# dluvizon/deephar

Measured on NVIDIA H100. Metric: frames/sec (256x256, 16-frame clips, b32), higher is better.
Workload: dtype bf16x3 split (fp32 accumulate, wgmma)

## Files before the change

deephar_b200/_ffi.py:

```python
import ctypes as C
import os

_HERE = os.path.dirname(os.path.abspath(__file__))
LIB_PATH = os.environ.get('DEEPHAR_B200_LIB') or os.path.join(_HERE, 'libdeephar_b200.so')


class DeepharB200Error(RuntimeError):
    pass


class dh_view(C.Structure):
    _fields_ = [('p', C.c_void_p), ('n', C.c_int32), ('h', C.c_int32), ('w', C.c_int32),
                ('c', C.c_int32), ('ld', C.c_int32)]


class dh_conv_desc(C.Structure):
    _fields_ = [('kh', C.c_int32), ('kw', C.c_int32), ('sh', C.c_int32), ('sw', C.c_int32),
                ('pad_same', C.c_int32), ('pre_relu', C.c_int32), ('post_relu', C.c_int32),
                ('n_res', C.c_int32),
                ('pre_scale', C.c_void_p), ('pre_shift', C.c_void_p),
                ('post_scale', C.c_void_p), ('post_shift', C.c_void_p),
                ('res', dh_view * 2),
                ('precision', C.c_int32), ('res_up2x', C.c_int32), ('pool_out', dh_view)]


class dh_frame_src(C.Structure):
    _fields_ = [('data', C.c_uint64), ('h', C.c_int32), ('w', C.c_int32), ('stride', C.c_int32),
                ('x0', C.c_int32), ('y0', C.c_int32), ('cw', C.c_int32), ('ch', C.c_int32), ('hflip', C.c_int32),
                ('kx_off', C.c_int32), ('ky_off', C.c_int32), ('kx_coef_off', C.c_int32), ('ky_coef_off', C.c_int32),
                ('ksx', C.c_int32), ('ksy', C.c_int32)]


class dh_frame_box(C.Structure):
    _fields_ = [('data', C.c_uint64), ('h', C.c_int32), ('w', C.c_int32), ('stride', C.c_int32),
                ('hflip', C.c_int32), ('objpos', C.c_double * 2), ('winsize', C.c_double * 2)]


FRAME_EMPTY, FRAME_TOO_LARGE, FRAME_BAD_BOX = 1, 2, 4


class dh_packed_w(C.Structure):
    _fields_ = [('hi', C.c_void_p), ('lo', C.c_void_p), ('cout_pad', C.c_int32), ('k', C.c_int32)]


class dh_conv_plan_info(C.Structure):
    _fields_ = [('path', C.c_int32), ('fallback', C.c_int32), ('workspace_bytes', C.c_int64),
                ('n_mtiles', C.c_int32), ('grid_x', C.c_int32), ('grid_y', C.c_int32), ('bn_cta', C.c_int32),
                ('n_kblocks', C.c_int32), ('stages', C.c_int32), ('cluster', C.c_int32), ('bm', C.c_int32),
                ('epi_tma', C.c_int32)]


class dh_clip_window(C.Structure):
    _fields_ = [('src', dh_view), ('dst', dh_view), ('ring', C.c_void_p)]


class dh_jpeg_image(C.Structure):
    _fields_ = [('data', C.c_int64), ('coef', C.c_int64 * 3), ('plane', C.c_int64 * 3), ('out', C.c_int64),
                ('h', C.c_int32), ('w', C.c_int32), ('ncomp', C.c_int32), ('hs', C.c_int32), ('vs', C.c_int32),
                ('mcus_x', C.c_int32), ('mcus_y', C.c_int32), ('bw', C.c_int32 * 3), ('bh', C.c_int32 * 3),
                ('qt', C.c_int32 * 3), ('dc', C.c_int32 * 3), ('ac', C.c_int32 * 3), ('nblocks', C.c_int32),
                ('pad', C.c_int32)]


class dh_jpeg_segment(C.Structure):
    _fields_ = [('begin', C.c_int64), ('end', C.c_int64), ('image', C.c_int32), ('mcu0', C.c_int32),
                ('mcus', C.c_int32), ('pad', C.c_int32)]


class dh_jpeg_huff(C.Structure):
    _fields_ = [('lut', C.c_uint16 * 512), ('maxcode', C.c_int32 * 18), ('valoff', C.c_int32 * 18),
                ('vals', C.c_uint8 * 256)]


class dh_jpeg_batch(C.Structure):
    _fields_ = [('images', C.c_uint64), ('segments', C.c_uint64), ('huff', C.c_uint64), ('qtab', C.c_uint64),
                ('data', C.c_uint64), ('coef', C.c_uint64), ('planes', C.c_uint64), ('out', C.c_uint64),
                ('status', C.c_uint64), ('coef_elems', C.c_int64), ('n_images', C.c_int32),
                ('n_segments', C.c_int32), ('max_blocks', C.c_int32), ('max_h', C.c_int32), ('max_w', C.c_int32),
                ('pad', C.c_int32)]


class dh_model_output_info(C.Structure):
# ... 140 lines not shown
```

deephar_b200/csrc/api.cu:

```cuda
#include <stdarg.h>
#include <string.h>
#include "common.cuh"

static thread_local char g_last_error[512] = "";

void dh_set_error(const char* fmt, ...) {
    va_list ap;
    va_start(ap, fmt);
    vsnprintf(g_last_error, sizeof(g_last_error), fmt, ap);
    va_end(ap);
}

extern "C" const char* dh_last_error(void) { return g_last_error; }

extern "C" int dh_version(void) { return 100; }

extern "C" int dh_ctx_create(dh_ctx** out, int device) {
    DH_CHECK_ARG(out != nullptr, "dh_ctx_create: out is NULL");
    int count = 0;
    cudaError_t e = cudaGetDeviceCount(&count);
    if (e != cudaSuccess || count == 0) {
        dh_set_error("dh_ctx_create: no CUDA device (%s) -- this library has no CPU fallback",
                     cudaGetErrorString(e));
        return e == cudaSuccess ? (int)cudaErrorNoDevice : (int)e;
    }
    DH_CHECK_ARG(device >= 0 && device < count, "dh_ctx_create: device %d out of range", device);
    cudaDeviceProp prop;
    e = cudaGetDeviceProperties(&prop, device);
    if (e != cudaSuccess) {
        dh_set_error("cudaGetDeviceProperties: %s", cudaGetErrorString(e));
        return (int)e;
    }
    if (prop.major != 9 || prop.minor != 0) {
        dh_set_error("dh_ctx_create: device %d is sm_%d%d; this build targets sm_90a (H100) only",
                     device, prop.major, prop.minor);
        return -2;
    }
    dh_ctx* c = new dh_ctx();
    c->device = device;
    c->num_sms = prop.multiProcessorCount;
    c->launches = 0;
    c->workspace = nullptr;
    c->workspace_bytes = 0;
    c->last_conv_path = 0;
    c->share_a = 1;
    c->sep_tma = 1;
    c->dbg = 0;
    c->pw_smallk = 1;
    c->dense_patch = 1;
    c->sam3d_stream = 1;
    c->fallbacks = 0;
    c->comm = nullptr;
    c->comm_rank = -1;
    c->comm_world = 0;
    *out = c;
    return 0;
}

extern "C" int dh_comm_destroy(dh_ctx* ctx);

extern "C" int dh_ctx_destroy(dh_ctx* ctx) {
    if (ctx && ctx->comm) dh_comm_destroy(ctx);
    delete ctx;
    return 0;
}

extern "C" int64_t dh_launch_count(dh_ctx* ctx, int reset) {
    if (!ctx) return -1;
    int64_t v = ctx->launches;
    if (reset) ctx->launches = 0;
    return v;
}

extern "C" int dh_set_option(dh_ctx* ctx, const char* name, int value) {
    DH_CHECK_ARG(ctx && name, "dh_set_option: NULL argument");
    if (!strcmp(name, "share_a")) { ctx->share_a = value; return 0; }
    if (!strcmp(name, "sep_tma")) { ctx->sep_tma = value; return 0; }
#ifdef DH_ABLATE
    if (!strcmp(name, "dbg")) { ctx->dbg = value; return 0; }
#endif
    if (!strcmp(name, "pw_smallk")) { ctx->pw_smallk = value; return 0; }
    if (!strcmp(name, "dense_patch")) { ctx->dense_patch = value; return 0; }
    if (!strcmp(name, "sam3d_stream")) { ctx->sam3d_stream = value; return 0; }
    dh_set_error("dh_set_option: unknown option %s", name);
    return -1;
}

extern "C" int dh_last_conv_path(dh_ctx* ctx) { return ctx ? ctx->last_conv_path : -1; }

extern "C" int64_t dh_fallback_count(dh_ctx* ctx, int reset) {
    if (!ctx) return -1;
    int64_t v = ctx->fallbacks;
    if (reset) ctx->fallbacks = 0;
    return v;
}

extern "C" int dh_set_workspace(dh_ctx* ctx, void* ptr, int64_t bytes) {
    DH_CHECK_ARG(ctx != nullptr, "dh_set_workspace: ctx is NULL");
    ctx->workspace = ptr;
    ctx->workspace_bytes = bytes;
    return 0;
}
```

deephar_b200/csrc/common.cuh:

```cuda
#pragma once
#include <cuda_runtime.h>
#include <stdint.h>
#include <stdio.h>
#include "../../include/deephar_b200.h"

struct dh_ctx {
    int device;
    int num_sms;
    int64_t launches;
    void* workspace;
    int64_t workspace_bytes;
    int last_conv_path;
    int share_a;
    int sep_tma;
    int pw_smallk;
    int sam3d_stream;
    int dense_patch;
    void* comm;
    int comm_rank, comm_world;
    int64_t fallbacks;
    int dbg;
};

void dh_set_error(const char* fmt, ...);

#define DH_CHECK_ARG(cond, ...)            \
    do {                                   \
        if (!(cond)) {                     \
            dh_set_error(__VA_ARGS__);     \
            return -1;                     \
        }                                  \
    } while (0)

#define DH_LAUNCH_EPILOGUE(ctx, nlaunch)                     \
    do {                                                     \
        (ctx)->launches += (nlaunch);                        \
        cudaError_t e__ = cudaGetLastError();                \
        if (e__ != cudaSuccess) {                            \
            dh_set_error("CUDA launch failed: %s (%s:%d)",   \
                         cudaGetErrorString(e__), __FILE__, __LINE__); \
            return (int)e__;                                 \
        }                                                    \
        return 0;                                            \
    } while (0)

static inline void dh_same_pad(int in, int k, int s, int* out, int* before) {
    int o = (in + s - 1) / s;
    int total = (o - 1) * s + k - in;
    if (total < 0) total = 0;
    *out = o;
// ... 84 lines not shown
```

deephar_b200/csrc/conv_api.cu:

```cuda
#include "tc_common.cuh"

namespace {

struct Choice {
    DhConvPath path;
    bool fallback;
    int64_t workspace_bytes;
    tc::PatchPlan patch;
    tc::SepPlan sep;
    tc::TcPlan tcp;
};

int choose_conv(const dh_ctx* ctx, const ConvParams& p, const dh_packed_w* packed, bool separable, int precision,
                Choice* c) {
    const bool packed_hi = packed && packed->hi;
    c->fallback = false;
    c->workspace_bytes = 0;
    if (separable) {
        DH_CHECK_ARG(!p.pool, "dh_sepconv2d_f32: pool_out is not supported by the separable kernels");
        if (packed_hi && dh_plan_sep_tma(ctx, p, packed, precision, &c->sep)) { c->path = DH_PATH_SEP_TMA; return 0; }
    } else {
        if (!p.up1 && !p.pool && dh_conv_smallk_ok(p)) { c->path = DH_PATH_SIMT; return 0; }
        if (ctx->pw_smallk && !p.up1 && dh_pw_smallk_supported(p)) { c->path = DH_PATH_PW_SMALLK; return 0; }
        DH_CHECK_ARG(!p.pool, "dh_conv2d_f32: pool_out is written by the wide pointwise kernel only (1x1, stride 1, "
// ... 58 lines not shown
    info->n_mtiles = P.n_mtiles;
    info->grid_x = tc::persistent_gx(ctx, pl.gy, P.n_mtiles);
    info->grid_y = pl.gy;
    info->bn_cta = P.bn_cta;
    info->n_kblocks = P.n_kblocks;
    info->cluster = pl.cluster;
    info->bm = tc::BM;
}

void simt_info(const SimtSchedule& g, dh_conv_plan_info* info) {
    info->bm = g.bm;
    info->n_mtiles = g.n_mtiles;
    info->grid_x = g.grid_x;
    info->grid_y = g.grid_y;
    info->bn_cta = g.bn_cta;
    info->n_kblocks = g.n_kblocks;
}

int plan_info(const dh_ctx* ctx, const ConvParams& p, bool separable, const Choice& c, dh_conv_plan_info* info) {
    DH_CHECK_ARG(info, "dh_conv_plan_info: NULL info");
    *info = dh_conv_plan_info{};
    info->path = c.path;
    info->fallback = c.fallback;
    info->workspace_bytes = c.workspace_bytes;
    if (c.path == DH_PATH_TC) {
        tc_info(ctx, c.tcp, c.tcp.k, info);
        info->stages = c.tcp.k.stages;
    }
    if (c.path == DH_PATH_SEP_TMA) {
        tc_info(ctx, c.sep, c.sep.k.t, info);
        info->bm = c.sep.k.bm;
        info->epi_tma = c.sep.k.epi_smem > 0;
    }
    if (c.path == DH_PATH_PATCH) tc_info(ctx, c.patch, c.patch.k.t, info);
    if (c.path == DH_PATH_PW_SMALLK) simt_info(dh_pw_smallk_schedule(p, ctx->num_sms), info);
    if (c.path == DH_PATH_SIMT)
        simt_info(dh_conv_simt_schedule(separable ? pointwise_stage(p, nullptr) : p, ctx->num_sms), info);
    return 0;
}

}

extern "C" int dh_conv2d_f32(dh_ctx* ctx, const dh_view* x, const float* w_hwio,
                             const dh_packed_w* packed, const dh_conv_desc* d, const dh_view* out,
                             void* stream) {
    ConvParams p;
    Choice c;
    int rc = plan_conv(ctx, x, nullptr, w_hwio, packed, d, out, false, &p, &c);
    return rc ? rc : launch_choice(ctx, p, c, false, (cudaStream_t)stream);
}

extern "C" int dh_sepconv2d_f32(dh_ctx* ctx, const dh_view* x, const float* w_dw, const float* w_pw,
                                const dh_packed_w* packed_pw, const dh_conv_desc* d,
                                const dh_view* out, void* stream) {
    ConvParams p;
    Choice c;
    int rc = plan_conv(ctx, x, w_dw, w_pw, packed_pw, d, out, true, &p, &c);
    return rc ? rc : launch_choice(ctx, p, c, true, (cudaStream_t)stream);
}

extern "C" int dh_conv2d_plan(dh_ctx* ctx, const dh_view* x, const float* w_hwio, const dh_packed_w* packed,
                              const dh_conv_desc* d, const dh_view* out, dh_conv_plan_info* info) {
    ConvParams p;
    Choice c;
    int rc = plan_conv(ctx, x, nullptr, w_hwio, packed, d, out, false, &p, &c);
    return rc ? rc : plan_info(ctx, p, false, c, info);
}
// ... 10 lines not shown
```

deephar_b200/csrc/conv_patch.cu:

```cuda
#include "tc_common.cuh"

namespace tcd {
using namespace tc;
using R = tc::Roles<2>;
constexpr int WARP_EPI0 = R::WARP_EPI0, WARP_TMA = R::WARP_TMA, WARP_PATCH = R::WARP_PATCH, NTHREADS = R::NTHREADS,
              REGS_PROD = R::REGS_PROD, REGS_EPI = R::REGS_EPI, REGS_CTRL = R::REGS_CTRL;

constexpr int NWG = 128;
constexpr int NA = 4;
constexpr int NB = 3;
constexpr int MAX_NP = 8;

template <bool LO>
__global__ void __launch_bounds__(NTHREADS, 1)
patch_dense_kernel(const __grid_constant__ PatchParams PP, const __grid_constant__ CUtensorMap map_hi,
                   const __grid_constant__ CUtensorMap map_lo, const __grid_constant__ CUtensorMap map_x) {
    const TcParams& P = PP.t;
    extern __shared__ __align__(1024) uint8_t smem_raw[];
    if (smem_u32(smem_raw) & 1023u) __trap();
    uint8_t* smem = smem_raw;
    const int tid = threadIdx.x;
    const int warp = tid >> 5, lane = tid & 31;
    constexpr bool want_lo = LO;
    const int b_bytes = P.bn_cta * 64;
    uint8_t* b_ring = smem + NA * 2 * A_BYTES;
    uint8_t* patch0 = b_ring + NB * 2 * b_bytes;
    uint64_t* bars = reinterpret_cast<uint64_t*>(patch0 + (size_t)PP.np * PP.patch_stride);
    float* post = reinterpret_cast<float*>(bars + 64);
    constexpr int NB_A = NA + 2 * NA;
    constexpr int NB_P = NB_A + 2 * NB;
    const uint32_t bar_full0 = smem_u32(bars), bar_empty0 = smem_u32(bars + NA), bar_fullb0 = smem_u32(bars + NB_A),
                   bar_emptyb0 = smem_u32(bars + NB_A + NB), bar_pfull0 = smem_u32(bars + NB_P),
                   bar_pempty0 = smem_u32(bars + NB_P + MAX_NP);
    const int n0 = blockIdx.y * P.bn_cta;
    const int nkb = P.n_kblocks;
    const int ntaps = PP.ntaps, ncb = PP.ncb, np = PP.np;

    if (warp == WARP_TMA && lane == 0) {
        tma_prefetch_desc(&map_hi);
        if (want_lo) tma_prefetch_desc(&map_lo);
        tma_prefetch_desc(&map_x);
        for (int s = 0; s < NA; ++s) {
            mbar_init(bar_full0 + 8 * s, (uint32_t)NWG);
            mbar_init(bar_empty0 + 16 * s, 1u);
            mbar_init(bar_empty0 + 16 * s + 8, 1u);
        }
        for (int s = 0; s < NB; ++s) {
            mbar_init(bar_fullb0 + 8 * s, 1);
            mbar_init(bar_emptyb0 + 8 * s, 1);
        }
        for (int s = 0; s < MAX_NP; ++s) {
            mbar_init(bar_pfull0 + 8 * s, 1);
            mbar_init(bar_pempty0 + 8 * s, ntaps == 1 ? (uint32_t)NWG : (uint32_t)(2 * NWG));
        }
        fence_barrier_init();
    }
    __syncthreads();

    const int tiles_mine = ((int)P.n_mtiles - (int)blockIdx.x + (int)gridDim.x - 1) / (int)gridDim.x;
    const int total_g = tiles_mine * nkb;
    const int n_patches = tiles_mine * ncb;
    const int rows_per_tile = BM / PP.tw;

    if (warp < WARP_EPI0) {
        reg_prod<REGS_PROD, R::LAUNCH_REGS>();
        const ConvParams& c = P.c;
        const int w = warp >> 2;
        const int tw = tid & (NWG - 1);
        const int ch4 = tw & 7;
        const int prow = tw >> 3;
        uint32_t poff[8];
        int yy[8], xx[8];
#pragma unroll
        for (int i = 0; i < 8; ++i) {
            const int m = prow + 16 * i;
            const int ty = m / PP.tw, tx = m - ty * PP.tw;
            const int f = ty / PP.ry, r = ty - f * PP.ry;
            poff[i] = (uint32_t)(((f * PP.pr + r * PP.sh) * PP.pc + tx * PP.sw) * (SBK * 4) + ch4 * 16);
            yy[i] = r * PP.sh - PP.pt;
            xx[i] = tx * PP.sw - PP.pl;
        }
        const uint32_t patch_s = smem_u32(patch0);
        const bool relu = c.pre_relu != 0, has_bn = c.pre_scale != nullptr;
        uint32_t aoff[8];
#pragma unroll
        for (int i = 0; i < 8; ++i) aoff[i] = swz64(prow + 16 * i, ch4 * 4);
        int tap = w % ntaps, p = w / ntaps;
        int cb = p % ncb, ti = p / ncb;
        int slot = p % np;
        uint32_t pphase = (uint32_t)(p / np) & 1u;
        int ky = tap / PP.kw, kx = tap - ky * PP.kw;
        int s = w % NA;
        uint32_t it = 0;
        int cb_loaded = -1, ti_masked = -1;
        float4 ps = make_float4(1.f, 1.f, 1.f, 1.f), pb = make_float4(0.f, 0.f, 0.f, 0.f);
        int y0 = 0;
        for (int g = w; g < total_g; g += 2) {
// ... 41 lines not shown
                }
                if (relu) {
                    t4.x = fmaxf(t4.x, 0.f); t4.y = fmaxf(t4.y, 0.f); t4.z = fmaxf(t4.z, 0.f); t4.w = fmaxf(t4.w, 0.f);
                }
                if (!((okmask >> i) & 1u)) t4 = make_float4(0.f, 0.f, 0.f, 0.f);
                uint32_t h0, l0, h1, l1;
                split2(t4.x, t4.y, h0, l0);
                split2(t4.z, t4.w, h1, l1);
                asm volatile("st.shared.v2.b32 [%0], {%1, %2};" ::"r"(a_hi + aoff[i]), "r"(h0), "r"(h1) : "memory");
                if (want_lo) asm volatile("st.shared.v2.b32 [%0], {%1, %2};" ::"r"(a_lo + aoff[i]), "r"(l0), "r"(l1) : "memory");
            }
            const bool last_of_patch = tap + 2 >= ntaps;
            if (last_of_patch) mbar_arrive(bar_pempty0 + 8 * slot);
            fence_proxy_async();
            mbar_arrive(bar_full0 + 8 * s);
            s += 2;
            if (s >= NA) { s -= NA; ++it; }
            tap += 2;
            kx += 2;
            while (tap >= ntaps) {
                tap -= ntaps;
                ++p;
                if (++cb == ncb) { cb = 0; ++ti; }
                if (++slot == np) { slot = 0; pphase ^= 1u; }
                ky = 0; kx = tap;
                if (kx >= PP.kw) { kx -= PP.kw; ky = 1; }
            }
            while (kx >= PP.kw) { kx -= PP.kw; ++ky; }
        }
    } else if (warp < WARP_TMA) {
        reg_inc<REGS_EPI>();
        stage_post<R::NEPI>(P, n0, post, tid - 32 * WARP_EPI0);
        const int wg = (warp - WARP_EPI0) >> 2, wt = tid - 32 * WARP_EPI0 - 128 * wg;
        pp_consumer<false, LO, NA, NB>(P, wg, wt, n0, tiles_mine, make_desc64(smem_u32(smem)), make_desc64(smem_u32(b_ring)),
                                       bar_full0, bar_empty0, bar_fullb0, bar_emptyb0, 0u, post, 0);
    } else {
        reg_dec<REGS_CTRL>();
        if (warp == WARP_TMA) {
            if (lane == 0) {
                const uint32_t tx = (uint32_t)(want_lo ? 2 : 1) * (uint32_t)b_bytes;
                for (int g = 0; g < total_g; ++g) {
                    const int p = g / ntaps, tap = g - p * ntaps;
                    const int cb = p % ncb;
                    const int kc = tap * P.c.Cin + cb * SBK;
                    const int sb = g % NB;
                    const uint32_t itb = (uint32_t)(g / NB);
                    if (itb >= 1) mbar_wait_relaxed(bar_emptyb0 + 8 * sb, (itb - 1) & 1, 0u);
                    const uint32_t full = bar_fullb0 + 8 * sb;
                    mbar_arrive_expect_tx(full, tx);
                    const uint32_t b_hi = smem_u32(b_ring + (size_t)sb * (2 * b_bytes));
                    const uint32_t b_lo = b_hi + (uint32_t)b_bytes;
                    tma_load_2d(b_hi, &map_hi, kc, n0, full);
                    if (want_lo) tma_load_2d(b_lo, &map_lo, kc, n0, full);
                }
            }
        } else if (warp == WARP_PATCH) {
            if (lane == 0) {
                for (int p = 0; p < n_patches; ++p) {
                    const int ti = p / ncb, cb = p - ti * ncb;
                    const int t = blockIdx.x + ti * gridDim.x;
                    const int grow = t * rows_per_tile;
                    const int nf = grow / PP.rows_per_frame;
                    const int y0 = grow - nf * PP.rows_per_frame;
                    const int slot = p % np;
                    const uint32_t u = (uint32_t)(p / np);
                    mbar_wait_relaxed(bar_pempty0 + 8 * slot, (u & 1u) ^ 1u, 0u);
                    const uint32_t pf = bar_pfull0 + 8 * slot;
                    mbar_arrive_expect_tx(pf, (uint32_t)PP.patch_bytes);
                    tma_load_4d(smem_u32(patch0 + (size_t)slot * PP.patch_stride), &map_x, cb * SBK, -PP.pl,
                                y0 * PP.sh - PP.pt, nf, pf);
                }
            }
        }
    }
}

static bool plan_geom(const ConvParams& p, PatchParams* g) {
    if (p.sh != 1 || p.sw != 1) return false;
    if (p.kh == 1 && p.kw == 1) {
// ... 20 lines not shown
    return true;
}

}

bool dh_plan_patch(const dh_ctx* ctx, const ConvParams& p, const dh_packed_w* packed, int precision, tc::PatchPlan* pl) {
    using namespace tc;
    using namespace tcd;
    if (!ctx->dense_patch || !packed->lo) return false;
    if (p.M < 1) return false;
    if ((p.Cin & 7) || (p.ldx & 3) || (reinterpret_cast<uintptr_t>(p.x) & 15) || !bn_pro_aligned(p)) return false;
    if (!packed_fits(packed, p.kh * p.kw * p.Cin, p.Cout)) return false;
    PatchParams& PP = pl->k;
    if (!plan_geom(p, &PP)) return false;
    if (PP.pc > 256 || PP.pr > 256 || PP.fn > 256) return false;
    if ((int64_t)PP.vh * PP.vw * p.ldx * 4 >= (1ll << 40)) return false;
    TcParams& P = PP.t;
    P.c = p;
    P.c.K = p.kh * p.kw * p.Cin;
    P.k_pad = packed->k;
    PP.ncb = (p.Cin + SBK - 1) / SBK;
    P.n_kblocks = PP.ncb * PP.ntaps;
    int gy;
    tile_n(p.Cout, &P.bn_cta, &gy);
    P.precision = (precision == 1) ? 1 : 3;
    P.ks = 0;
    P.n_mtiles = (p.M + BM - 1) / BM;
    P.stages = 2;
    P.dbg = 0;
    PP.sh = 1; PP.sw = 1;
    PP.mask = (p.pre_scale != nullptr && PP.ntaps > 1) ? 1 : 0;
    PP.patch_bytes = SBK * 4 * PP.pc * PP.pr * PP.fn;
    PP.patch_stride = (PP.patch_bytes + 1023) / 1024 * 1024;
    const size_t fixed = (size_t)NA * 2 * A_BYTES + (size_t)NB * 2 * P.bn_cta * 64 + 512 + POST_SMEM;
    const int np = (int)((SMEM_LIMIT - fixed) / (size_t)PP.patch_stride);
    if (np < 2) return false;
    PP.np = np > MAX_NP ? MAX_NP : np;
    pl->w = packed;
    pl->gy = gy;
    pl->smem = fixed + (size_t)PP.np * PP.patch_stride;
    pl->cluster = false;
    return true;
}

int dh_launch_patch(const dh_ctx* ctx, const tc::PatchPlan& pl, cudaStream_t s) {
    using namespace tc;
    using namespace tcd;
    const PatchParams& PP = pl.k;
    const ConvParams& c = PP.t.c;
    const dh_packed_w* w = pl.w;
    const int vn = PP.ntaps == 1 ? 1 : c.N;
    CUtensorMap map_hi, map_lo, map_x;
    if (!make_map_w(&map_hi, w->hi, w->k, w->cout_pad, SBK, PP.t.bn_cta) ||
        !make_map_w(&map_lo, w->lo, w->k, w->cout_pad, SBK, PP.t.bn_cta) ||
        !make_map_x(&map_x, c.x, c.ldx, c.Cin, PP.vw, PP.vh, vn, PP.pc, PP.pr, PP.fn)) {
        dh_set_error("dh_launch_patch: cuTensorMapEncodeTiled failed");
        return -1;
    }
    return pick<true, false>(PP.t.precision == 3, [&](auto lo) {
        return launch_persistent<patch_dense_kernel<lo()>>("dh_launch_patch", ctx, pl, PP.t.n_mtiles, NTHREADS, s,
                                                           map_hi, map_lo, map_x);
    });
}
```

deephar_b200/csrc/tc_common.cuh:

```cuda
#pragma once
#include <cuda.h>
#include <cuda_bf16.h>
#include <type_traits>
#include "common.cuh"
#include "conv_params.cuh"

namespace tc {


constexpr int BM = 128;
constexpr int BK = 64;
constexpr int NPROD = 256;
constexpr int MAX_BN_CTA = 96;
constexpr int ACC_N = MAX_BN_CTA / 2;
constexpr int MH = BM / 64;
constexpr int BM64 = 64;
constexpr int MAX_BN_CTA64 = 144;
constexpr int bn_max(int bm) { return bm == BM64 ? MAX_BN_CTA64 : MAX_BN_CTA; }
template <int Q, int NPW = 2>
struct Roles {
    static constexpr int EPQ = Q;
    static constexpr int NEPI = 128 * Q;
    static constexpr int WARP_EPI0 = 4 * NPW;
    static constexpr int WARP_TMA = WARP_EPI0 + 4 * Q, WARP_PATCH = WARP_TMA + 2;
// ... 11 lines not shown
    ConvParams c;
    int n_kblocks;
    int bn_cta;
    int stages;
    int precision;
    int ks;
    int k_pad;
    int n_mtiles;
    int dbg;
};

struct SepParams {
    TcParams t;
    int patch_stride;
    int patch_bytes;
    int ry, fn;
    int bm;
    int epi_smem;
    int dbg;
};

struct PatchParams {
    TcParams t;
    int np, patch_stride, patch_bytes;
    int ntaps, ncb;
    int tw;
    int ry, fn;
    int pc, pr;
    int rows_per_frame;
    int kw;
    int pt, pl, sh, sw;
    int vh, vw;
    int mask;
};

__device__ __forceinline__ void mbar_wait_relaxed(uint32_t bar, uint32_t parity, uint32_t ns) {
    uint32_t ok;
    for (;;) {
        asm volatile(
            "{\n .reg .pred p;\n mbarrier.try_wait.parity.shared::cta.b64 p, [%1], %2;\n selp.u32 %0, 1, 0, p;\n}"
            : "=r"(ok)
            : "r"(bar), "r"(parity)
            : "memory");
        if (ok) break;
        if (ns) __nanosleep(ns);
    }
}
__device__ __forceinline__ void fence_proxy_async() { asm volatile("fence.proxy.async.shared::cta;" ::: "memory"); }

__device__ __forceinline__ void tma_load_2d(uint32_t dst, const CUtensorMap* map, int c0, int c1, uint32_t bar) {
    asm volatile(
        "cp.async.bulk.tensor.2d.shared::cluster.global.mbarrier::complete_tx::bytes [%0], [%1, {%2, %3}], [%4];"
        ::"r"(dst), "l"(map), "r"(c0), "r"(c1), "r"(bar)
        : "memory");
}
__device__ __forceinline__ void tma_prefetch_desc(const CUtensorMap* map) {
    asm volatile("prefetch.tensormap [%0];" ::"l"(map) : "memory");
}
__device__ __forceinline__ void tma_store_2d(const CUtensorMap* map, uint32_t src, int c0, int c1) {
    asm volatile("cp.async.bulk.tensor.2d.global.shared::cta.bulk_group [%0, {%2, %3}], [%1];"
                 ::"l"(map), "r"(src), "r"(c0), "r"(c1)
                 : "memory");
}
__device__ __forceinline__ void bulk_commit() { asm volatile("cp.async.bulk.commit_group;" ::: "memory"); }
__device__ __forceinline__ void bulk_wait_read() { asm volatile("cp.async.bulk.wait_group.read 0;" ::: "memory"); }
__device__ __forceinline__ void bulk_s2peer(uint32_t dst_cluster, uint32_t src_cta, uint32_t bytes, uint32_t bar_cluster) {
// ... 98 lines not shown
__device__ __forceinline__ void tma_prefetch_4d(const CUtensorMap* map, int c0, int c1, int c2, int c3) {
    asm volatile("cp.async.bulk.prefetch.tensor.4d.L2.global [%0, {%1, %2, %3, %4}];"
                 ::"l"(map), "r"(c0), "r"(c1), "r"(c2), "r"(c3) : "memory");
}

__device__ __forceinline__ uint64_t make_desc64(uint32_t smem_addr) {
    return (uint64_t)((smem_addr >> 4) & 0x3FFF) | (1ull << 16) | ((uint64_t)(512 >> 4) << 32) | (2ull << 62);
}
__device__ __forceinline__ uint32_t swz64(int row, int k) {
    return (uint32_t)(row * 64 + ((((k >> 3) ^ ((row >> 1) & 3)) << 4) | ((k & 7) << 1)));
}

__device__ __forceinline__ float4 lds128(uint32_t a) {
    float4 v;
    asm volatile("ld.shared.v4.f32 {%0, %1, %2, %3}, [%4];" : "=f"(v.x), "=f"(v.y), "=f"(v.z), "=f"(v.w) : "r"(a) : "memory");
    return v;
}

__device__ __forceinline__ void wait_stage_free(uint32_t bar_empty0, int s, uint32_t it, uint32_t ns = 0) {
    if (it >= 1) mbar_wait_relaxed(bar_empty0 + 16 * s + 8 * ((it - 1) & 1), ((it - 1) >> 1) & 1, ns);
}


template <int N, int MHT, int ACCN>
__device__ __forceinline__ void acc_fence_all(float (&acc)[MHT][ACCN]) {
#pragma unroll
    for (int h = 0; h < MHT; ++h)
#pragma unroll
        for (int i = 0; i < N / 2; ++i) acc_fence(acc[h][i]);
}

template <int N, int NK16, bool LO, int MHT, int ACCN>
__device__ __forceinline__ void wg_issue_kblock(float (&acc)[MHT][ACCN], uint64_t da, uint32_t a_half16, uint32_t alo16,
                                                uint64_t db, uint32_t blo16, bool first) {
    wgmma_fence();
#pragma unroll
    for (int k = 0; k < NK16; ++k) {
        const uint32_t acc0 = (first && k == 0) ? 0u : 1u;
#pragma unroll
        for (int h = 0; h < MHT; ++h) {
            const uint64_t a = da + (uint64_t)(h * a_half16 + 2 * k);
            wgmma_bf16<N>(acc[h], a, db + 2 * k, acc0);
            if (LO) {
                wgmma_bf16<N>(acc[h], a + alo16, db + 2 * k, 1u);
                wgmma_bf16<N>(acc[h], a, db + blo16 + 2 * k, 1u);
            }
        }
    }
    wgmma_commit();
}

template <int N, int NK16, bool LO, int MHT, int ACCN, class Stage, class Release>
__device__ __forceinline__ void wg_tile_n(float (&acc)[MHT][ACCN], int nkb, uint32_t a_half16, uint32_t alo16,
                                          uint32_t blo16, bool mma, Stage& stage, Release& release) {
    for (int kb = 0; kb < nkb; ++kb) {
        uint64_t da, db;
        stage(kb, da, db);
        if (mma) {
            acc_fence_all<N>(acc);
            wg_issue_kblock<N, NK16, LO>(acc, da, a_half16, alo16, db, blo16, kb == 0);
        }
        wgmma_wait<1>();
        acc_fence_all<N>(acc);
        if (kb > 0) release(kb - 1);
    }
    wgmma_wait<0>();
    acc_fence_all<N>(acc);
    release(nkb - 1);
}

template <int NK16, bool LO, int MHT, int ACCN, class Stage, class Release>
__device__ __forceinline__ void wg_tile(int bn, float (&acc)[MHT][ACCN], int nkb, uint32_t a_half16, uint32_t alo16,
                                        uint32_t blo16, bool mma, Stage&& stage, Release&& release) {
    if constexpr (ACCN == MAX_BN_CTA64 / 2) {
        wg_tile_n<MAX_BN_CTA64, NK16, LO>(acc, nkb, a_half16, alo16, blo16, mma, stage, release);
    } else {
        switch (bn) {
        case 16: wg_tile_n<16, NK16, LO>(acc, nkb, a_half16, alo16, blo16, mma, stage, release); break;
        case 32: wg_tile_n<32, NK16, LO>(acc, nkb, a_half16, alo16, blo16, mma, stage, release); break;
        case 48: wg_tile_n<48, NK16, LO>(acc, nkb, a_half16, alo16, blo16, mma, stage, release); break;
        case 64: wg_tile_n<64, NK16, LO>(acc, nkb, a_half16, alo16, blo16, mma, stage, release); break;
        case 80: wg_tile_n<80, NK16, LO>(acc, nkb, a_half16, alo16, blo16, mma, stage, release); break;
        default: wg_tile_n<96, NK16, LO>(acc, nkb, a_half16, alo16, blo16, mma, stage, release); break;
        }
    }
}

__device__ __forceinline__ void pp_pass(int wg) { asm volatile("bar.arrive %0, 256;" ::"r"(6 + wg) : "memory"); }
__device__ __forceinline__ void pp_wait(int wg) { asm volatile("bar.sync %0, 256;" ::"r"(7 - wg) : "memory"); }

__device__ __forceinline__ void wg_release(uint32_t bar, int wg, int wt, bool remote, uint32_t peer) {
    asm volatile("bar.sync %0, 128;" ::"r"(4 + wg) : "memory");
    if (wt == 0) {
        mbar_arrive(bar);
        if (remote) mbar_arrive_cluster(mapa_peer(bar, peer));
    }
}

__device__ __forceinline__ float2 ldg2(const float* p) { return __ldg(reinterpret_cast<const float2*>(p)); }

constexpr int post_smem(int bm) { return 2 * bn_max(bm) * 4; }
constexpr int POST_SMEM = post_smem(BM);
template <int NEPI, int BNMAX = MAX_BN_CTA>
__device__ __forceinline__ void stage_post(const TcParams& P, int n0, float* post, int ct) {
    const ConvParams& c = P.c;
    if (c.post_scale) {
        for (int j = ct; j < P.bn_cta; j += NEPI) {
            const int co = n0 + j;
            post[j] = co < c.Cout ? __ldg(c.post_scale + co) : 0.f;
            post[BNMAX + j] = co < c.Cout ? __ldg(c.post_shift + co) : 0.f;
        }
    }
    asm volatile("bar.sync 2, %0;" ::"n"(NEPI) : "memory");
}

__device__ __forceinline__ void prefetch_l2(const float* p) { asm volatile("prefetch.global.L2 [%0];" ::"l"(p)); }
// ... 339 lines not shown
```

include/deephar_b200.h:

```cpp
#ifndef DEEPHAR_B200_H
#define DEEPHAR_B200_H

#include <stdint.h>

#ifdef __cplusplus
extern "C" {
#endif

typedef struct dh_view {
    float*  p;
    int32_t n, h, w, c;
    int32_t ld;
} dh_view;

typedef struct dh_conv_desc {
    int32_t kh, kw, sh, sw;
    int32_t pad_same;
    int32_t pre_relu;
    int32_t post_relu;
    int32_t n_res;
    const float* pre_scale;
    const float* pre_shift;
    const float* post_scale;
    const float* post_shift;
// ... 13 lines not shown

int         dh_ctx_create(dh_ctx** out, int device);
int         dh_ctx_destroy(dh_ctx* ctx);
const char* dh_last_error(void);
int         dh_version(void);
int64_t     dh_launch_count(dh_ctx* ctx, int reset);
int         dh_set_workspace(dh_ctx* ctx, void* ptr, int64_t bytes);
int         dh_set_option(dh_ctx* ctx, const char* name, int value);

int dh_tc_cout_pad(int cout);
int dh_tc_k_pad(int k);
int dh_last_conv_path(dh_ctx* ctx);
int64_t dh_fallback_count(dh_ctx* ctx, int reset);

int dh_conv2d_f32(dh_ctx* ctx, const dh_view* x, const float* w_hwio, const dh_packed_w* packed,
                  const dh_conv_desc* d, const dh_view* out, void* stream);

int dh_sepconv2d_f32(dh_ctx* ctx, const dh_view* x, const float* w_dw, const float* w_pw,
                     const dh_packed_w* packed_pw, const dh_conv_desc* d, const dh_view* out,
                     void* stream);

typedef struct dh_conv_plan_info {
    int32_t path;
    int32_t fallback;
    int64_t workspace_bytes;
    int32_t n_mtiles;
    int32_t grid_x, grid_y;
    int32_t bn_cta;
    int32_t n_kblocks;
    int32_t stages;
    int32_t cluster;
    int32_t bm;
    int32_t epi_tma;
} dh_conv_plan_info;
int dh_conv2d_plan(dh_ctx* ctx, const dh_view* x, const float* w_hwio, const dh_packed_w* packed,
                   const dh_conv_desc* d, const dh_view* out, dh_conv_plan_info* info);
int dh_sepconv2d_plan(dh_ctx* ctx, const dh_view* x, const float* w_dw, const float* w_pw,
                      const dh_packed_w* packed_pw, const dh_conv_desc* d, const dh_view* out,
                      dh_conv_plan_info* info);

int dh_maxpool2d_f32(dh_ctx* ctx, const dh_view* x, int kh, int kw, int sh, int sw, int pad_same,
                     const dh_view* out, void* stream);
int dh_upsample2x_add_f32(dh_ctx* ctx, const dh_view* a, const dh_view* b, const dh_view* out,
                          void* stream);
int dh_add_n_f32(dh_ctx* ctx, const dh_view* in, int n_in, const float* scale, const float* shift,
                 int relu, const dh_view* out, void* stream);

int dh_softargmax2d_f32(dh_ctx* ctx, const dh_view* h, const dh_view* d, float alpha,
                        int conf_on_prob, float* out_pose, float* out_conf,
                        const dh_view* prob_out, void* stream);

int dh_softargmax2d_ctx_f32(dh_ctx* ctx, const dh_view* h, int nj, int n_ctx, float alpha_mix,
                            float* out_pose, float* out_vis, void* stream);

int dh_softargmax3d_f32(dh_ctx* ctx, const dh_view* h, int nj, int depth_maps,
                        float* out_pose, float* out_vis, void* stream);

int dh_softargmax3d_ex_f32(dh_ctx* ctx, const dh_view* h, int nj, int depth_maps, float vis_scale,
                           float* out_pose, float* out_vis, const dh_view* prob_out, void* stream);

int dh_kron_pool_f32(dh_ctx* ctx, const dh_view* p, const dh_view* z, float* out, void* stream);

int dh_zeropad2d_f32(dh_ctx* ctx, const dh_view* x, int top, int left, const dh_view* out, void* stream);
int dh_maxmin_pool2d_f32(dh_ctx* ctx, const dh_view* x, const dh_view* out, void* stream);
int dh_global_maxmin_softmax_f32(dh_ctx* ctx, const dh_view* x, float* out, void* stream);
int dh_mask_mul_f32(dh_ctx* ctx, const float* p, const float* c, int64_t rows, int dim, float* out,
// ... 159 lines not shown
```

Measured before the change: 4068.

## Convert patch once per channel block and slice taps via shifted wgmma descriptors

Adds a 'taps' mode to the dense patch conv kernel. Producer warps now BN/ReLU/mask and split each input patch into bf16 hi/lo once per channel block, writing it into a non-swizzled ring. Consumers then address each kernel tap by offsetting the wgmma A descriptor instead of rebuilding an im2col A tile per tap. This removes the per-tap staging and conversion work and frees shared memory for a deeper B ring (6 stages). The cost is a new barrier protocol, a different smem layout whose non-swizzled A reads may cause bank conflicts, and the mode only applies for W of 64 or 128 with a single frame.

```diff
diff --git a/deephar_b200/_ffi.py b/deephar_b200/_ffi.py
--- a/deephar_b200/_ffi.py
+++ b/deephar_b200/_ffi.py
@@ -47,7 +47,7 @@
     _fields_ = [('path', C.c_int32), ('fallback', C.c_int32), ('workspace_bytes', C.c_int64),
                 ('n_mtiles', C.c_int32), ('grid_x', C.c_int32), ('grid_y', C.c_int32), ('bn_cta', C.c_int32),
                 ('n_kblocks', C.c_int32), ('stages', C.c_int32), ('cluster', C.c_int32), ('bm', C.c_int32),
-                ('epi_tma', C.c_int32)]
+                ('epi_tma', C.c_int32), ('patch_taps', C.c_int32)]
 
 
 class dh_clip_window(C.Structure):
diff --git a/deephar_b200/csrc/api.cu b/deephar_b200/csrc/api.cu
--- a/deephar_b200/csrc/api.cu
+++ b/deephar_b200/csrc/api.cu
@@ -48,6 +48,7 @@
     c->dbg = 0;
     c->pw_smallk = 1;
     c->dense_patch = 1;
+    c->patch_taps = 1;
     c->sam3d_stream = 1;
     c->fallbacks = 0;
     c->comm = nullptr;
@@ -81,6 +82,7 @@
 #endif
     if (!strcmp(name, "pw_smallk")) { ctx->pw_smallk = value; return 0; }
     if (!strcmp(name, "dense_patch")) { ctx->dense_patch = value; return 0; }
+    if (!strcmp(name, "patch_taps")) { ctx->patch_taps = value; return 0; }
     if (!strcmp(name, "sam3d_stream")) { ctx->sam3d_stream = value; return 0; }
     dh_set_error("dh_set_option: unknown option %s", name);
     return -1;
diff --git a/deephar_b200/csrc/common.cuh b/deephar_b200/csrc/common.cuh
--- a/deephar_b200/csrc/common.cuh
+++ b/deephar_b200/csrc/common.cuh
@@ -16,6 +16,7 @@
     int pw_smallk;
     int sam3d_stream;
     int dense_patch;
+    int patch_taps;
     void* comm;
     int comm_rank, comm_world;
     int64_t fallbacks;
diff --git a/deephar_b200/csrc/conv_api.cu b/deephar_b200/csrc/conv_api.cu
--- a/deephar_b200/csrc/conv_api.cu
+++ b/deephar_b200/csrc/conv_api.cu
@@ -114,7 +114,10 @@
         info->bm = c.sep.k.bm;
         info->epi_tma = c.sep.k.epi_smem > 0;
     }
-    if (c.path == DH_PATH_PATCH) tc_info(ctx, c.patch, c.patch.k.t, info);
+    if (c.path == DH_PATH_PATCH) {
+        tc_info(ctx, c.patch, c.patch.k.t, info);
+        info->patch_taps = c.patch.k.taps;
+    }
     if (c.path == DH_PATH_PW_SMALLK) simt_info(dh_pw_smallk_schedule(p, ctx->num_sms), info);
     if (c.path == DH_PATH_SIMT)
         simt_info(dh_conv_simt_schedule(separable ? pointwise_stage(p, nullptr) : p, ctx->num_sms), info);
diff --git a/deephar_b200/csrc/conv_patch.cu b/deephar_b200/csrc/conv_patch.cu
--- a/deephar_b200/csrc/conv_patch.cu
+++ b/deephar_b200/csrc/conv_patch.cu
@@ -9,9 +9,70 @@
 constexpr int NWG = 128;
 constexpr int NA = 4;
 constexpr int NB = 3;
+constexpr int TAPS_NB = 6;
+constexpr int MAX_NB = TAPS_NB;
+constexpr int NC = 2;
 constexpr int MAX_NP = 8;
-
-template <bool LO>
+constexpr int NB_A = NA + 2 * NA;
+constexpr int NB_P = NB_A + 2 * MAX_NB;
+static_assert(2 * NC <= NB_A && NB_P + 2 * MAX_NP <= 64, "the barriers fit their 512 bytes");
+
+__device__ __forceinline__ uint64_t make_desc_ns(uint32_t smem_addr, uint32_t lbo) {
+    return (uint64_t)((smem_addr >> 4) & 0x3FFF) | ((uint64_t)((lbo >> 4) & 0x3FFF) << 16) | ((uint64_t)(128 >> 4) << 32);
+}
+
+template <bool LO, int TNB>
+__device__ __forceinline__ void taps_consumer(const PatchParams& PP, int wg, int wt, int n0, int tiles_mine,
+                                              uint32_t cring, uint32_t b_ring, uint32_t bars, const float* post) {
+    const TcParams& P = PP.t;
+    const int nkb = P.n_kblocks, ntaps = PP.ntaps, kw = PP.kw, pc = PP.pc;
+    const uint32_t bar_cfull0 = bars, bar_cempty0 = bars + 8 * NC, bar_fullb0 = bars + 8 * NB_A,
+                   bar_emptyb0 = bars + 8 * (NB_A + MAX_NB);
+    const uint32_t lbo = (uint32_t)PP.crows * 16;
+    const uint32_t stb16 = (uint32_t)(2 * P.bn_cta * 64) >> 4, blo16 = (uint32_t)(P.bn_cta * 64) >> 4;
+    const uint32_t a_half16 = PP.tw == 128 ? 64u : (uint32_t)pc;
+    const uint64_t dbase_b = make_desc64(b_ring);
+    float acc[MH][ACC_N];
+    for (int ti = wg; ti < tiles_mine; ti += 2) {
+        const int g0 = ti * nkb, m0 = ((int)blockIdx.x + ti * (int)gridDim.x) * BM;
+        if (ti > 0) pp_wait(wg);
+        wg_prefetch_res(P, m0, n0, wt);
+        int p = ti * PP.ncb - 1;
+        int tap = 0, kx = 0;
+        uint32_t toff = 0;
+        bool first_tap = false;
+        const bool more = ti + 1 < tiles_mine;
+        wg_tile<SBK / 16, LO>(
+            P.bn_cta, acc, nkb, a_half16, (uint32_t)PP.crows * 4, blo16, true,
+            [&](int kb, uint64_t& da, uint64_t& db) {
+                const int g = g0 + kb, sb = g % TNB;
+                first_tap = tap == 0;
+                if (first_tap) {
+                    ++p;
+                    mbar_wait(bar_cfull0 + 8 * (p % NC), (uint32_t)(p / NC) & 1);
+                }
+                mbar_wait(bar_fullb0 + 8 * sb, (uint32_t)(g / TNB) & 1);
+                if (kb == nkb - 1 && more) pp_pass(wg);
+                da = make_desc_ns(cring + (uint32_t)(p % NC) * (uint32_t)(PP.crows * 128) + 16 * toff, lbo);
+                db = dbase_b + (uint64_t)((uint32_t)sb * stb16);
+                ++toff;
+                if (++kx == kw) { kx = 0; toff += (uint32_t)(pc - kw); }
+                if (++tap == ntaps) { tap = 0; toff = 0; }
+            },
+            [&](int kb) {
+                asm volatile("bar.sync %0, 128;" ::"r"(4 + wg) : "memory");
+                if (wt == 0) {
+                    if (kb == nkb - 1) mbar_arrive(bar_cempty0 + 8 * (p % NC));
+                    else if (first_tap) mbar_arrive(bar_cempty0 + 8 * ((p - 1) % NC));
+                    mbar_arrive(bar_emptyb0 + 8 * ((g0 + kb) % TNB));
+                }
+            },
+            (uint32_t)PP.crows * 2);
+        wg_epilogue(P, acc, m0, n0, wt, post);
+    }
+}
+
+template <bool LO, int TNB>
 __global__ void __launch_bounds__(NTHREADS, 1)
 patch_dense_kernel(const __grid_constant__ PatchParams PP, const __grid_constant__ CUtensorMap map_hi,
                    const __grid_constant__ CUtensorMap map_lo, const __grid_constant__ CUtensorMap map_x) {
@@ -23,15 +84,16 @@
     const int warp = tid >> 5, lane = tid & 31;
     constexpr bool want_lo = LO;
     const int b_bytes = P.bn_cta * 64;
-    uint8_t* b_ring = smem + NA * 2 * A_BYTES;
-    uint8_t* patch0 = b_ring + NB * 2 * b_bytes;
+    constexpr bool TAPS = TNB > 0;
+    constexpr int nb = TAPS ? TNB : NB;
+    uint8_t* b_ring = smem + PP.a_bytes;
+    uint8_t* patch0 = b_ring + (size_t)nb * 2 * b_bytes;
     uint64_t* bars = reinterpret_cast<uint64_t*>(patch0 + (size_t)PP.np * PP.patch_stride);
     float* post = reinterpret_cast<float*>(bars + 64);
-    constexpr int NB_A = NA + 2 * NA;
-    constexpr int NB_P = NB_A + 2 * NB;
     const uint32_t bar_full0 = smem_u32(bars), bar_empty0 = smem_u32(bars + NA), bar_fullb0 = smem_u32(bars + NB_A),
-                   bar_emptyb0 = smem_u32(bars + NB_A + NB), bar_pfull0 = smem_u32(bars + NB_P),
+                   bar_emptyb0 = smem_u32(bars + NB_A + MAX_NB), bar_pfull0 = smem_u32(bars + NB_P),
                    bar_pempty0 = smem_u32(bars + NB_P + MAX_NP);
+    const uint32_t bar_cfull0 = bar_full0, bar_cempty0 = smem_u32(bars + NC);
     const int n0 = blockIdx.y * P.bn_cta;
     const int nkb = P.n_kblocks;
     const int ntaps = PP.ntaps, ncb = PP.ncb, np = PP.np;
@@ -40,12 +102,19 @@
         tma_prefetch_desc(&map_hi);
         if (want_lo) tma_prefetch_desc(&map_lo);
         tma_prefetch_desc(&map_x);
-        for (int s = 0; s < NA; ++s) {
-            mbar_init(bar_full0 + 8 * s, (uint32_t)NWG);
-            mbar_init(bar_empty0 + 16 * s, 1u);
-            mbar_init(bar_empty0 + 16 * s + 8, 1u);
-        }
-        for (int s = 0; s < NB; ++s) {
+        if (TAPS) {
+            for (int s = 0; s < NC; ++s) {
+                mbar_init(bar_cfull0 + 8 * s, (uint32_t)(2 * NWG));
+                mbar_init(bar_cempty0 + 8 * s, 1u);
+            }
+        } else {
+            for (int s = 0; s < NA; ++s) {
+                mbar_init(bar_full0 + 8 * s, (uint32_t)NWG);
+                mbar_init(bar_empty0 + 16 * s, 1u);
+                mbar_init(bar_empty0 + 16 * s + 8, 1u);
+            }
+        }
+        for (int s = 0; s < nb; ++s) {
             mbar_init(bar_fullb0 + 8 * s, 1);
             mbar_init(bar_emptyb0 + 8 * s, 1);
         }
@@ -62,7 +131,71 @@
     const int n_patches = tiles_mine * ncb;
     const int rows_per_tile = BM / PP.tw;
 
-    if (warp < WARP_EPI0) {
+    if (TAPS && warp < WARP_EPI0) {
+        reg_prod<REGS_PROD, R::LAUNCH_REGS>();
+        const ConvParams& c = P.c;
+        const int ch4 = tid & 7, q = tid >> 3;
+        const int npix = PP.pr * PP.pc, pc = PP.pc;
+        const uint32_t lbo = (uint32_t)PP.crows * 16, lo_off = 4 * lbo;
+        const uint32_t st_off = (uint32_t)(ch4 >> 1) * lbo + (uint32_t)(ch4 & 1) * 8 + (uint32_t)q * 16;
+        const uint32_t ld_off = (uint32_t)(q * (SBK * 4) + ch4 * 16);
+        const uint32_t patch_s = smem_u32(patch0), cring = smem_u32(smem);
+        const bool relu = c.pre_relu != 0, has_bn = c.pre_scale != nullptr;
+        const int q_r = q / pc, q_c = q - q_r * pc;
+        float4 ps = make_float4(1.f, 1.f, 1.f, 1.f), pb = make_float4(0.f, 0.f, 0.f, 0.f);
+        int cb = 0, ti = 0, slot = 0, cs = 0, cb_loaded = -1;
+        uint32_t pphase = 0, cuse = 0;
+        for (int p = 0; p < n_patches; ++p) {
+            if (has_bn && cb != cb_loaded) {
+                cb_loaded = cb;
+                const int ci = cb * SBK + ch4 * 4;
+                if (ci < c.Cin) {
+                    ps = __ldg(reinterpret_cast<const float4*>(c.pre_scale + ci));
+                    pb = __ldg(reinterpret_cast<const float4*>(c.pre_shift + ci));
+                } else {
+                    ps = make_float4(0.f, 0.f, 0.f, 0.f);
+                    pb = make_float4(0.f, 0.f, 0.f, 0.f);
+                }
+            }
+            int ylo = 0;
+            if (PP.mask) {
+                const int t = blockIdx.x + ti * gridDim.x;
+                ylo = (t * PP.ry) % PP.rows_per_frame - PP.pt;
+            }
+            mbar_wait(bar_pfull0 + 8 * slot, pphase);
+            if (cuse >= 1) mbar_wait_relaxed(bar_cempty0 + 8 * cs, (cuse - 1) & 1u, 0u);
+            const uint32_t src = patch_s + (uint32_t)slot * (uint32_t)PP.patch_stride + ld_off;
+            const uint32_t dst = cring + (uint32_t)cs * (uint32_t)(PP.crows * 128) + st_off;
+            int r = q_r, cc = q_c;
+#pragma unroll 4
+            for (int i = q; i < npix; i += 32) {
+                float4 t4 = lds128(src + (uint32_t)(i - q) * (SBK * 4));
+                if (has_bn) {
+                    t4.x = fmaf(t4.x, ps.x, pb.x); t4.y = fmaf(t4.y, ps.y, pb.y);
+                    t4.z = fmaf(t4.z, ps.z, pb.z); t4.w = fmaf(t4.w, ps.w, pb.w);
+                }
+                if (relu) {
+                    t4.x = fmaxf(t4.x, 0.f); t4.y = fmaxf(t4.y, 0.f); t4.z = fmaxf(t4.z, 0.f); t4.w = fmaxf(t4.w, 0.f);
+                }
+                if (PP.mask && !((unsigned)(ylo + r) < (unsigned)PP.vh && (unsigned)(cc - PP.pl) < (unsigned)PP.vw))
+                    t4 = make_float4(0.f, 0.f, 0.f, 0.f);
+                uint32_t h0, l0, h1, l1;
+                split2(t4.x, t4.y, h0, l0);
+                split2(t4.z, t4.w, h1, l1);
+                const uint32_t a = dst + (uint32_t)(i - q) * 16;
+                asm volatile("st.shared.v2.b32 [%0], {%1, %2};" ::"r"(a), "r"(h0), "r"(h1) : "memory");
+                if (want_lo) asm volatile("st.shared.v2.b32 [%0], {%1, %2};" ::"r"(a + lo_off), "r"(l0), "r"(l1) : "memory");
+                cc += 32;
+                if (cc >= pc) { cc -= pc; ++r; }
+            }
+            mbar_arrive(bar_pempty0 + 8 * slot);
+            fence_proxy_async();
+            mbar_arrive(bar_cfull0 + 8 * cs);
+            if (++slot == np) { slot = 0; pphase ^= 1u; }
+            if (++cs == NC) { cs = 0; ++cuse; }
+            if (++cb == ncb) { cb = 0; ++ti; }
+        }
+    } else if (warp < WARP_EPI0) {
         reg_prod<REGS_PROD, R::LAUNCH_REGS>();
         const ConvParams& c = P.c;
         const int w = warp >> 2;
@@ -170,8 +303,12 @@
         reg_inc<REGS_EPI>();
         stage_post<R::NEPI>(P, n0, post, tid - 32 * WARP_EPI0);
         const int wg = (warp - WARP_EPI0) >> 2, wt = tid - 32 * WARP_EPI0 - 128 * wg;
-        pp_consumer<false, LO, NA, NB>(P, wg, wt, n0, tiles_mine, make_desc64(smem_u32(smem)), make_desc64(smem_u32(b_ring)),
-                                       bar_full0, bar_empty0, bar_fullb0, bar_emptyb0, 0u, post, 0);
+        if constexpr (TAPS)
+            taps_consumer<LO, nb>(PP, wg, wt, n0, tiles_mine, smem_u32(smem), smem_u32(b_ring), smem_u32(bars), post);
+        else
+            pp_consumer<false, LO, NA, NB>(P, wg, wt, n0, tiles_mine, make_desc64(smem_u32(smem)),
+                                           make_desc64(smem_u32(b_ring)), bar_full0, bar_empty0, bar_fullb0, bar_emptyb0,
+                                           0u, post, 0);
     } else {
         reg_dec<REGS_CTRL>();
         if (warp == WARP_TMA) {
@@ -181,8 +318,8 @@
                     const int p = g / ntaps, tap = g - p * ntaps;
                     const int cb = p % ncb;
                     const int kc = tap * P.c.Cin + cb * SBK;
-                    const int sb = g % NB;
-                    const uint32_t itb = (uint32_t)(g / NB);
+                    const int sb = g % nb;
+                    const uint32_t itb = (uint32_t)(g / nb);
                     if (itb >= 1) mbar_wait_relaxed(bar_emptyb0 + 8 * sb, (itb - 1) & 1, 0u);
                     const uint32_t full = bar_fullb0 + 8 * sb;
                     mbar_arrive_expect_tx(full, tx);
@@ -269,13 +406,31 @@
     PP.mask = (p.pre_scale != nullptr && PP.ntaps > 1) ? 1 : 0;
     PP.patch_bytes = SBK * 4 * PP.pc * PP.pr * PP.fn;
     PP.patch_stride = (PP.patch_bytes + 1023) / 1024 * 1024;
-    const size_t fixed = (size_t)NA * 2 * A_BYTES + (size_t)NB * 2 * P.bn_cta * 64 + 512 + POST_SMEM;
-    const int np = (int)((SMEM_LIMIT - fixed) / (size_t)PP.patch_stride);
-    if (np < 2) return false;
-    PP.np = np > MAX_NP ? MAX_NP : np;
+    const size_t b_stage = (size_t)2 * P.bn_cta * 64, other = 512 + POST_SMEM;
+    PP.taps = 0;
+    if (ctx->patch_taps && PP.ntaps > 1 && PP.fn == 1 && (p.W == 128 || p.W == 64)) {
+        const int npix = PP.pr * PP.pc;
+        PP.crows = npix + ((10 - npix % 8) % 8);
+        const size_t a_bytes = ((size_t)NC * PP.crows * 128 + 1023) / 1024 * 1024;
+        const size_t need = a_bytes + 2 * (size_t)PP.patch_stride + NB * b_stage + other;
+        if (need <= SMEM_LIMIT) {
+            PP.nb = need + (TAPS_NB - NB) * b_stage <= SMEM_LIMIT ? TAPS_NB : NB;
+            const size_t np = (SMEM_LIMIT - a_bytes - PP.nb * b_stage - other) / (size_t)PP.patch_stride;
+            PP.np = np > MAX_NP ? MAX_NP : (int)np;
+            PP.a_bytes = (int)a_bytes;
+            PP.taps = 1;
+        }
+    }
+    if (!PP.taps) {
+        PP.a_bytes = NA * 2 * A_BYTES;
+        PP.nb = NB;
+        const int np = (int)((SMEM_LIMIT - PP.a_bytes - NB * b_stage - other) / (size_t)PP.patch_stride);
+        if (np < 2) return false;
+        PP.np = np > MAX_NP ? MAX_NP : np;
+    }
     pl->w = packed;
     pl->gy = gy;
-    pl->smem = fixed + (size_t)PP.np * PP.patch_stride;
+    pl->smem = (size_t)PP.a_bytes + PP.nb * b_stage + (size_t)PP.np * PP.patch_stride + other;
     pl->cluster = false;
     return true;
 }
@@ -295,7 +450,9 @@
         return -1;
     }
     return pick<true, false>(PP.t.precision == 3, [&](auto lo) {
-        return launch_persistent<patch_dense_kernel<lo()>>("dh_launch_patch", ctx, pl, PP.t.n_mtiles, NTHREADS, s,
-                                                           map_hi, map_lo, map_x);
+        return pick<0, NB, TAPS_NB>(PP.taps ? PP.nb : 0, [&](auto tnb) {
+            return launch_persistent<patch_dense_kernel<lo(), tnb()>>("dh_launch_patch", ctx, pl, PP.t.n_mtiles,
+                                                                      NTHREADS, s, map_hi, map_lo, map_x);
+        });
     });
 }
diff --git a/deephar_b200/csrc/tc_common.cuh b/deephar_b200/csrc/tc_common.cuh
--- a/deephar_b200/csrc/tc_common.cuh
+++ b/deephar_b200/csrc/tc_common.cuh
@@ -67,6 +67,10 @@
     int pt, pl, sh, sw;
     int vh, vw;
     int mask;
+    int taps;
+    int crows;
+    int nb;
+    int a_bytes;
 };
 
 __device__ __forceinline__ void mbar_wait_relaxed(uint32_t bar, uint32_t parity, uint32_t ns) {
@@ -231,14 +235,14 @@
 
 template <int N, int NK16, bool LO, int MHT, int ACCN>
 __device__ __forceinline__ void wg_issue_kblock(float (&acc)[MHT][ACCN], uint64_t da, uint32_t a_half16, uint32_t alo16,
-                                                uint64_t db, uint32_t blo16, bool first) {
+                                                uint64_t db, uint32_t blo16, bool first, uint32_t a_k16) {
     wgmma_fence();
 #pragma unroll
     for (int k = 0; k < NK16; ++k) {
         const uint32_t acc0 = (first && k == 0) ? 0u : 1u;
 #pragma unroll
         for (int h = 0; h < MHT; ++h) {
-            const uint64_t a = da + (uint64_t)(h * a_half16 + 2 * k);
+            const uint64_t a = da + (uint64_t)(h * a_half16 + a_k16 * k);
             wgmma_bf16<N>(acc[h], a, db + 2 * k, acc0);
             if (LO) {
                 wgmma_bf16<N>(acc[h], a + alo16, db + 2 * k, 1u);
@@ -251,13 +255,13 @@
 
 template <int N, int NK16, bool LO, int MHT, int ACCN, class Stage, class Release>
 __device__ __forceinline__ void wg_tile_n(float (&acc)[MHT][ACCN], int nkb, uint32_t a_half16, uint32_t alo16,
-                                          uint32_t blo16, bool mma, Stage& stage, Release& release) {
+                                          uint32_t blo16, bool mma, Stage& stage, Release& release, uint32_t a_k16) {
     for (int kb = 0; kb < nkb; ++kb) {
         uint64_t da, db;
         stage(kb, da, db);
         if (mma) {
             acc_fence_all<N>(acc);
-            wg_issue_kblock<N, NK16, LO>(acc, da, a_half16, alo16, db, blo16, kb == 0);
+            wg_issue_kblock<N, NK16, LO>(acc, da, a_half16, alo16, db, blo16, kb == 0, a_k16);
         }
         wgmma_wait<1>();
         acc_fence_all<N>(acc);
@@ -270,17 +274,17 @@
 
 template <int NK16, bool LO, int MHT, int ACCN, class Stage, class Release>
 __device__ __forceinline__ void wg_tile(int bn, float (&acc)[MHT][ACCN], int nkb, uint32_t a_half16, uint32_t alo16,
-                                        uint32_t blo16, bool mma, Stage&& stage, Release&& release) {
+                                        uint32_t blo16, bool mma, Stage&& stage, Release&& release, uint32_t a_k16 = 2) {
     if constexpr (ACCN == MAX_BN_CTA64 / 2) {
-        wg_tile_n<MAX_BN_CTA64, NK16, LO>(acc, nkb, a_half16, alo16, blo16, mma, stage, release);
+        wg_tile_n<MAX_BN_CTA64, NK16, LO>(acc, nkb, a_half16, alo16, blo16, mma, stage, release, a_k16);
     } else {
         switch (bn) {
-        case 16: wg_tile_n<16, NK16, LO>(acc, nkb, a_half16, alo16, blo16, mma, stage, release); break;
-        case 32: wg_tile_n<32, NK16, LO>(acc, nkb, a_half16, alo16, blo16, mma, stage, release); break;
-        case 48: wg_tile_n<48, NK16, LO>(acc, nkb, a_half16, alo16, blo16, mma, stage, release); break;
-        case 64: wg_tile_n<64, NK16, LO>(acc, nkb, a_half16, alo16, blo16, mma, stage, release); break;
-        case 80: wg_tile_n<80, NK16, LO>(acc, nkb, a_half16, alo16, blo16, mma, stage, release); break;
-        default: wg_tile_n<96, NK16, LO>(acc, nkb, a_half16, alo16, blo16, mma, stage, release); break;
+        case 16: wg_tile_n<16, NK16, LO>(acc, nkb, a_half16, alo16, blo16, mma, stage, release, a_k16); break;
+        case 32: wg_tile_n<32, NK16, LO>(acc, nkb, a_half16, alo16, blo16, mma, stage, release, a_k16); break;
+        case 48: wg_tile_n<48, NK16, LO>(acc, nkb, a_half16, alo16, blo16, mma, stage, release, a_k16); break;
+        case 64: wg_tile_n<64, NK16, LO>(acc, nkb, a_half16, alo16, blo16, mma, stage, release, a_k16); break;
+        case 80: wg_tile_n<80, NK16, LO>(acc, nkb, a_half16, alo16, blo16, mma, stage, release, a_k16); break;
+        default: wg_tile_n<96, NK16, LO>(acc, nkb, a_half16, alo16, blo16, mma, stage, release, a_k16); break;
         }
     }
 }
diff --git a/include/deephar_b200.h b/include/deephar_b200.h
--- a/include/deephar_b200.h
+++ b/include/deephar_b200.h
@@ -69,6 +69,7 @@
     int32_t cluster;
     int32_t bm;
     int32_t epi_tma;
+    int32_t patch_taps;
 } dh_conv_plan_info;
 int dh_conv2d_plan(dh_ctx* ctx, const dh_view* x, const float* w_hwio, const dh_packed_w* packed,
                    const dh_conv_desc* d, const dh_view* out, dh_conv_plan_info* info);
```

After: 4102, median of 6. About the same (+0.8%).
